# ForeverFancy/GVFDiffusion

Measured on AMD Instinct MI355X. Metric: 4D frames/sec (800x800x24f, 256k Gaussians) + DiT denoise steps/sec, higher is better.
Workload: dtype f32; 1 GPU; BASELINE configs[1]: single-GPU HIP rasteriser, one 4D sample per step = 24 frames x 800x800, 262144 Gaussians + per-frame deltas (fused activations), SH degree 2, mip 2D filter, white bg; gaussians=262144, resolution=800, sh_degree=2, parallelism=sample-sharded x1, samples_in_flight=2

## Files before the change

### gvfdiffusion_amd/csrc/rast.hip

```cpp
#include <atomic>
#include <cstdlib>
#include <vector>
#include "rast_common.h"
#include "gvf_sort.h"

namespace {

#ifndef GVF_PRE_FB
#define GVF_PRE_FB 4
#endif
constexpr int PRE_FB = GVF_PRE_FB;
#ifndef GVF_PRE_WAVE_FB
#define GVF_PRE_WAVE_FB 6
#endif
constexpr int PRE_WAVES = PRE_THREADS / GVF_WAVE;
constexpr int PRE_WAVE_FB = GVF_PRE_WAVE_FB;

struct PreParams {
    int P, M, deg, H, W, mode;
    int gx, gy;
    float kernel_size, scale_modifier;
    int fused;
    GvfGaussianActivation act;
    int n_delta;
    int upstream_binning;
    int F;
    int delta_lds;
};

__global__ __launch_bounds__(256) void activate_kernel(GvfGaussianActivation a, int P, int M,
                                                       const float* __restrict__ xyz_raw,
                                                       const float* __restrict__ features_dc,
                                                       const float* __restrict__ scaling_raw,
                                                       const float* __restrict__ rotation_raw,
                                                       const float* __restrict__ opacity_raw,
                                                       const float* __restrict__ delta, float* __restrict__ means3D,
                                                       float* __restrict__ scales, float* __restrict__ rotations,
                                                       float* __restrict__ shs, float* __restrict__ opacities) {
    int i = blockIdx.x * blockDim.x + threadIdx.x;
    if (i >= P) return;
    const float* d = delta ? delta + 14 * (size_t)i : nullptr;
    ActGaussian g = activate_one(i, a, xyz_raw, scaling_raw, rotation_raw, opacity_raw, d);
    for (int k = 0; k < 3; ++k) { means3D[3 * (size_t)i + k] = g.p[k]; scales[3 * (size_t)i + k] = g.s[k]; }
    for (int k = 0; k < 4; ++k) rotations[4 * (size_t)i + k] = g.q[k];
    opacities[i] = g.op;
    for (int m = 0; m < M; ++m)
        for (int c = 0; c < 3; ++c) {
            float v = features_dc[((size_t)i * M + m) * 3 + c];
            shs[((size_t)i * M + m) * 3 + c] = d ? v + g.drgb[c] : v;
        }
}

constexpr int ACT_MAX_SLICES = 16;
struct ActSlices { int n; int di[ACT_MAX_SLICES]; };
__global__ __launch_bounds__(256) void activate_cov_kernel(GvfGaussianActivation a, float scale_modifier, int P, ActSlices sl,
                                                           const float* __restrict__ xyz_raw, const float* __restrict__ scaling_raw,
                                                           const float* __restrict__ rotation_raw, const float* __restrict__ opacity_raw,
                                                           const float* __restrict__ delta, float4* __restrict__ rec3d,
                                                           const uint32_t* __restrict__ slot_of ,
                                                           const float* __restrict__ sh, int sh_floats, float* __restrict__ sh_by_slot) {
    const int i = blockIdx.x * blockDim.x + threadIdx.x;
    if (i >= P) return;
    const size_t dst = slot_of != nullptr ? (size_t)slot_of[i] : (size_t)i;
    if (sh_by_slot != nullptr && blockIdx.y == 0)
        for (int k = 0; k < sh_floats; ++k) sh_by_slot[dst * sh_floats + k] = sh[(size_t)i * sh_floats + k];
    const int di = sl.di[blockIdx.y];
    const float* d = (delta != nullptr && di >= 0) ? delta + ((size_t)di * P + i) * 14 : nullptr;
    const ActGaussian g = activate_one(i, a, xyz_raw, scaling_raw, rotation_raw, opacity_raw, d);
    float c6[6];
    cov3d_from_scale_rot(g.s, scale_modifier, g.q, c6);
    float4* r = rec3d + 4 * ((size_t)blockIdx.y * P + dst);
    r[0] = make_float4(g.p[0], g.p[1], g.p[2], g.op);
    r[1] = make_float4(c6[0], c6[1], c6[2], c6[3]);
    r[2] = make_float4(c6[4], c6[5], g.drgb[0], g.drgb[1]);
    r[3] = make_float4(g.drgb[2], 0.f, 0.f, 0.f);
}

__device__ __forceinline__ float ln_upper(float z) {
    const uint32_t b = __float_as_uint(z);
    const int e = (int)(b >> 23) - 127;
    const float m = __uint_as_float((b & 0x7fffffu) | 0x3f800000u);
    float L = (m - 1.0f) * 1.4426951f;
    L = fminf(L, 0.32192809f + (m - 1.25f) * 1.1541561f);
    L = fminf(L, 0.5849625f + (m - 1.5f) * 0.96179669f);
    L = fminf(L, 0.80735492f + (m - 1.75f) * 0.8243972f);
    L = fminf(L, 1.0f + (m - 2.0f) * 0.72134752f);
    return ((float)e + (L + 1e-5f)) * 0.69314724f;
}

__device__ __forceinline__ float2 cull_extent(float ca, float cb, float cc, float op) {
    if (op < 1.0f / 255.0f) return make_float2(-1.0f, -1.0f);
    const float det = ca * cc - cb * cb;
    const float inf = __builtin_inff();
    if (!(det > 0.0f) || !(ca > 0.0f) || !(cc > 0.0f)) return make_float2(inf, inf);
    const float tau = 2.0f * ln_upper(255.0f * op) * 1.001f + 1e-3f;
    const float inv = 1.0f / det;
    return make_float2(sqrtf(tau * cc * inv) * 1.001f + 0.01f, sqrtf(tau * ca * inv) * 1.001f + 0.01f);
}

__device__ __forceinline__ void tight_range(float c, float h, int lo, int hi, int n, int& t0, int& t1) {
    if (h < 0.0f) { t0 = lo; t1 = lo; return; }
    const float a = fminf(fmaxf(ceilf((c - h - (float)(TILE - 1)) / (float)TILE), 0.0f), (float)n);
    const float b = fminf(fmaxf(floorf((c + h) / (float)TILE) + 1.0f, 0.0f), (float)n);
    t0 = max((int)a, lo);
    t1 = min((int)b, hi);
    if (t1 < t0) t1 = t0;
}

__device__ __forceinline__ TileRect tight_rect(TileRect r, float px, float py, float hx, float hy, int gx, int gy) {
    TileRect t;
    tight_range(px, hx, r.x0, r.x1, gx, t.x0, t.x1);
    tight_range(py, hy, r.y0, r.y1, gy, t.y0, t.y1);
    return t;
}

template <bool SHARED, bool WAVE_FRAMES = false>
__global__ __launch_bounds__(PRE_THREADS) void preprocess_kernel(
    PreParams pp, const GvfRastFrame* __restrict__ frames, const float* __restrict__ a0,
    const float* __restrict__ a1, const float* __restrict__ a2, const float* __restrict__ a3,
    const float* __restrict__ sh, const float* __restrict__ colors_precomp,
    const float* __restrict__ cov3D_precomp, const float* __restrict__ delta, float4* __restrict__ splats,
    uint32_t* __restrict__ tiles_touched,
    int32_t* __restrict__ radii, uint32_t* __restrict__ block_sums, uint4* __restrict__ binrec,
    const uint32_t* __restrict__ bin_slot ) {
    static_assert(!(SHARED && WAVE_FRAMES), "the shared-activation launch keeps the 256-Gaussian mapping");
    extern __shared__ __attribute__((aligned(16))) float sh_lds[];
    constexpr int PRE_GPB = WAVE_FRAMES ? GVF_WAVE : PRE_THREADS;
    const int t = threadIdx.x;
    const int P = pp.P, M = pp.M;
    const int nbx = (P + PRE_THREADS - 1) / PRE_THREADS;
    const int bx = blockIdx.x, by = blockIdx.y;
    const int row = WAVE_FRAMES ? (t & (GVF_WAVE - 1)) : t;
    const int i = bx * PRE_GPB + row;

    const int sh_stride = M * 3;
    if (sh != nullptr) {
        const size_t span0 = (size_t)bx * PRE_GPB * sh_stride;
        const int nvalid = min(PRE_GPB, P - bx * PRE_GPB);
        const int total = nvalid * sh_stride;
        const float4* src4 = reinterpret_cast<const float4*>(sh + span0);
        float4* dst4 = reinterpret_cast<float4*>(sh_lds);
        const int n4 = total >> 2;
        for (int k = t; k < n4; k += PRE_THREADS) dst4[k] = src4[k];
        for (int k = (n4 << 2) + t; k < total; k += PRE_THREADS) sh_lds[k] = sh[span0 + k];
    }
    __syncthreads();

  const uint32_t my_slot = (bin_slot != nullptr && i < P) ? bin_slot[i] : (uint32_t)i;
  ActRaw raw = {};
  if (WAVE_FRAMES && pp.fused && i < P) raw = activate_raw(i, pp.act, a0, a1, a2, a3);
  const int f_first = WAVE_FRAMES ? by * (PRE_WAVES * PRE_WAVE_FB) + __builtin_amdgcn_readfirstlane(t >> 6) : by * PRE_FB;
  constexpr int F_STEP = WAVE_FRAMES ? PRE_WAVES : 1, F_COUNT = WAVE_FRAMES ? PRE_WAVE_FB : PRE_FB;
#pragma unroll 1
  for (int ff = 0; ff < F_COUNT; ++ff) {
    const int f = f_first + ff * F_STEP;
    if (f >= pp.F) break;
    const GvfRastFrame* fr = frames + f;
    uint32_t touched = 0;
    int radius_out = 0;
    float4 gA = make_float4(0.f, 0.f, 0.f, 0.f), gB = gA, gC = gA;
    TileRect rect = {0, 0, 0, 0};

    if (i < P) {
        float p[3], s[3], q[4], op, dadd[3] = {0.f, 0.f, 0.f};
        float c6s[6];
        if (SHARED) {
            const float4* r3 = reinterpret_cast<const float4*>(a0) + 4 * ((size_t)fr->reserved[0] * P + i);
            const float4 r0 = r3[0], r1 = r3[1], r2 = r3[2], r3v = r3[3];
            p[0] = r0.x; p[1] = r0.y; p[2] = r0.z; op = r0.w;
            c6s[0] = r1.x; c6s[1] = r1.y; c6s[2] = r1.z; c6s[3] = r1.w; c6s[4] = r2.x; c6s[5] = r2.y;
            dadd[0] = r2.z; dadd[1] = r2.w; dadd[2] = r3v.x;
        } else if (pp.fused) {
            const int di = fr->delta_index;
            const float* d = (delta != nullptr && di >= 0) ? delta + ((size_t)di * P + i) * 14 : nullptr;
            ActGaussian g;
            if (WAVE_FRAMES) {
                float dl[14];
#pragma unroll
                for (int k = 0; k < 14; ++k) dl[k] = d ? d[k] : 0.0f;
                g = activate_finish(raw, pp.act, dl, d != nullptr);
            } else {
                g = activate_one(i, pp.act, a0, a1, a2, a3, d);
            }
#pragma unroll
            for (int k = 0; k < 3; ++k) { p[k] = g.p[k]; s[k] = g.s[k]; dadd[k] = g.drgb[k]; }
#pragma unroll
            for (int k = 0; k < 4; ++k) q[k] = g.q[k];
            op = g.op;
        } else {
#pragma unroll
            for (int k = 0; k < 3; ++k) p[k] = a0[3 * (size_t)i + k];
            if (cov3D_precomp == nullptr) {
#pragma unroll
                for (int k = 0; k < 3; ++k) s[k] = a1[3 * (size_t)i + k];
#pragma unroll
                for (int k = 0; k < 4; ++k) q[k] = a2[4 * (size_t)i + k];
            }
            op = a3[i];
        }

        float pv[3];
        xform43(fr->viewmatrix, p, pv);
        bool vis = pv[2] > 0.2f;
        if (vis) {
            float ph[4];
            xform44(fr->projmatrix, p, ph);
            float pw = 1.0f / (ph[3] + 0.0000001f);
            float projx = ph[0] * pw, projy = ph[1] * pw;

            float c6[6];
            if (SHARED) {
#pragma unroll
                for (int k = 0; k < 6; ++k) c6[k] = c6s[k];
            } else if (!pp.fused && cov3D_precomp != nullptr) {
#pragma unroll
                for (int k = 0; k < 6; ++k) c6[k] = cov3D_precomp[6 * (size_t)i + k];
            } else {
                cov3d_from_scale_rot(s, pp.scale_modifier, q, c6);
            }

            const float tanfovx = fr->tanfovx, tanfovy = fr->tanfovy;
            float focal_x = (float)pp.W / (2.0f * tanfovx);
            float focal_y = (float)pp.H / (2.0f * tanfovy);
            float limx = 1.3f * tanfovx, limy = 1.3f * tanfovy;
            float txtz = pv[0] / pv[2], tytz = pv[1] / pv[2];
            float tx = fminf(limx, fmaxf(-limx, txtz)) * pv[2];
            float ty = fminf(limy, fmaxf(-limy, tytz)) * pv[2];
            float tz = pv[2];
            float J00 = focal_x / tz, J02 = -(focal_x * tx) / (tz * tz);
            float J11 = focal_y / tz, J12 = -(focal_y * ty) / (tz * tz);
            float A0[3], A1[3];
#pragma unroll
            for (int c = 0; c < 3; ++c) {
                float w0 = fr->viewmatrix[c * 4 + 0], w1 = fr->viewmatrix[c * 4 + 1], w2 = fr->viewmatrix[c * 4 + 2];
                A0[c] = J00 * w0 + J02 * w2;
                A1[c] = J11 * w1 + J12 * w2;
            }
            float S[3][3] = {{c6[0], c6[1], c6[2]}, {c6[1], c6[3], c6[4]}, {c6[2], c6[4], c6[5]}};
            float B0[3], B1[3];
#pragma unroll
            for (int c = 0; c < 3; ++c) {
                B0[c] = A0[0] * S[0][c] + A0[1] * S[1][c] + A0[2] * S[2][c];
                B1[c] = A1[0] * S[0][c] + A1[1] * S[1][c] + A1[2] * S[2][c];
            }
            float cxx = B0[0] * A0[0] + B0[1] * A0[1] + B0[2] * A0[2];
            float cxy = B0[0] * A1[0] + B0[1] * A1[1] + B0[2] * A1[2];
            float cyy = B1[0] * A1[0] + B1[1] * A1[1] + B1[2] * A1[2];

            float coef = 1.0f;
            if (pp.mode == GVF_RAST_MODE_MIP) {
                float det0 = fmaxf(1e-6f, cxx * cyy - cxy * cxy);
                float det1 = fmaxf(1e-6f, (cxx + pp.kernel_size) * (cyy + pp.kernel_size) - cxy * cxy);
                coef = sqrtf(det0 / (det1 + 1e-6f) + 1e-6f);
                if (det0 <= 1e-6f || det1 <= 1e-6f) coef = 0.0f;
                cxx += pp.kernel_size;
                cyy += pp.kernel_size;
            } else {
                cxx += 0.3f;
                cyy += 0.3f;
            }
            float det = cxx * cyy - cxy * cxy;
            if (det != 0.0f) {
                float det_inv = 1.f / det;
                float ca = cyy * det_inv, cb = -cxy * det_inv, cc = cxx * det_inv;
                float mid = 0.5f * (cxx + cyy);
                float lam1 = mid + sqrtf(fmaxf(0.1f, mid * mid - det));
                float lam2 = mid - sqrtf(fmaxf(0.1f, mid * mid - det));
                float my_radius = ceilf(3.f * sqrtf(fmaxf(lam1, lam2)));
                float px = ((projx + 1.0f) * (float)pp.W - 1.0f) * 0.5f;
                float py = ((projy + 1.0f) * (float)pp.H - 1.0f) * 0.5f;
                TileRect r = get_rect(px, py, my_radius, pp.gx, pp.gy);
                uint32_t cnt = (uint32_t)((r.x1 - r.x0) * (r.y1 - r.y0));
                if (cnt != 0) {
                    float rgb[3];
                    if (colors_precomp != nullptr) {
                        rgb[0] = colors_precomp[3 * (size_t)i + 0];
                        rgb[1] = colors_precomp[3 * (size_t)i + 1];
                        rgb[2] = colors_precomp[3 * (size_t)i + 2];
                    } else {
                        sh_to_rgb(pp.deg, sh_lds + row * sh_stride, dadd, p, fr->campos, rgb);
                    }
                    radius_out = (int)my_radius;
                    const float2 ext = cull_extent(ca, cb, cc, op * coef);
                    if (!pp.upstream_binning) {
                        r = tight_rect(r, px, py, ext.x, ext.y, pp.gx, pp.gy);
                        cnt = (uint32_t)((r.x1 - r.x0) * (r.y1 - r.y0));
                    }
                    touched = cnt;
                    rect = r;
                    gA = make_float4(px, py, ca * CONIC_K1, cb * CONIC_K2);
                    gB = make_float4(cc * CONIC_K1, op * coef, rgb[0], rgb[1]);
                    gC = make_float4(rgb[2], pv[2], ext.x, ext.y);
                }
            }
        }
        const size_t o = (size_t)f * P + i;
        if (!WAVE_FRAMES && tiles_touched != nullptr) tiles_touched[o] = touched;
        if (radii != nullptr) {
            const uint32_t* gid_of = SHARED ? reinterpret_cast<const uint32_t*>(a1) : nullptr;
            radii[gid_of != nullptr ? (size_t)f * P + gid_of[i] : o] = radius_out;
        }
        if (binrec != nullptr) {
            binrec[(size_t)f * P + my_slot] = make_uint4((uint32_t)rect.x0 | ((uint32_t)rect.y0 << 16),
                                                         (uint32_t)rect.x1 | ((uint32_t)rect.y1 << 16), __float_as_uint(gC.y), 0u);
        }
    }

    const int lj = t & 3;
    float4* qbase = splats + 4 * ((size_t)f * P + (size_t)(i & ~3));
#define GVF_QB(v_, k_) __builtin_bit_cast(float, __builtin_amdgcn_mov_dpp(__builtin_bit_cast(int, (v_)), (k_) * 0x55, 0xF, 0xF, true))
#define GVF_QSTORE(k_)                                                                                          \
    {                                                                                                       \
        const int tk = __builtin_amdgcn_mov_dpp((int)touched, (k_) * 0x55, 0xF, 0xF, true);                 \
        float4 o4;                                                                                          \
        { const float a = GVF_QB(gA.x, k_), b = GVF_QB(gB.x, k_), c = GVF_QB(gC.x, k_); o4.x = lj == 0 ? a : (lj == 1 ? b : (lj == 2 ? c : 0.f)); } \
        { const float a = GVF_QB(gA.y, k_), b = GVF_QB(gB.y, k_), c = GVF_QB(gC.y, k_); o4.y = lj == 0 ? a : (lj == 1 ? b : (lj == 2 ? c : 0.f)); } \
        { const float a = GVF_QB(gA.z, k_), b = GVF_QB(gB.z, k_), c = GVF_QB(gC.z, k_); o4.z = lj == 0 ? a : (lj == 1 ? b : (lj == 2 ? c : 0.f)); } \
        { const float a = GVF_QB(gA.w, k_), b = GVF_QB(gB.w, k_), c = GVF_QB(gC.w, k_); o4.w = lj == 0 ? a : (lj == 1 ? b : (lj == 2 ? c : 0.f)); } \
        if (tk != 0) qbase[4 * (k_) + lj] = o4;                                                             \
    }
    GVF_QSTORE(0) GVF_QSTORE(1) GVF_QSTORE(2) GVF_QSTORE(3)
#undef GVF_QSTORE
#undef GVF_QB

    if (!WAVE_FRAMES && block_sums != nullptr) {
        const unsigned lane = t & 63, w = t >> 6;
        uint32_t incl = gvf_wave_incl_scan(touched, lane);
        __shared__ uint32_t wsum[PRE_THREADS / GVF_WAVE];
        __syncthreads();
        if (lane == 63) wsum[w] = incl;
        __syncthreads();
        if (t == 0) block_sums[(size_t)f * nbx + bx] = wsum[0] + wsum[1] + wsum[2] + wsum[3];
    }
  }
}

__global__ __launch_bounds__(1024) void scan_sums_kernel(uint32_t* __restrict__ block_sums, int nb, int F,
                                                         uint32_t* __restrict__ frame_base ,
                                                         uint32_t* __restrict__ num_rendered ,
                                                         uint32_t* __restrict__ total_out, uint32_t max_rendered) {
    __shared__ uint32_t wsum[16];
    __shared__ uint32_t carry_s;
    const int t = threadIdx.x;
    const unsigned lane = t & 63, w = t >> 6;
    const int n = nb * F;
    if (t == 0) carry_s = 0;
    __syncthreads();
    for (int base = 0; base < n; base += 1024) {
        int j = base + t;
        uint32_t v = j < n ? block_sums[j] : 0u;
        uint32_t incl = gvf_wave_incl_scan(v, lane);
        if (lane == 63) wsum[w] = incl;
        __syncthreads();
        uint32_t wbase = 0, tot = 0;
        for (unsigned k = 0; k < 16; ++k) { if (k < w) wbase += wsum[k]; tot += wsum[k]; }
        uint32_t carry = carry_s;
        uint32_t excl = carry + wbase + incl - v;
        if (j < n) {
            block_sums[j] = excl;
            if (j % nb == 0) frame_base[j / nb] = excl;
        }
        __syncthreads();
        if (t == 0) carry_s = carry + tot;
        __syncthreads();
    }
    if (t == 0) { frame_base[F] = carry_s; *total_out = carry_s > max_rendered ? 0u : carry_s; }
    __syncthreads();
    for (int f = t; f < F; f += 1024) num_rendered[f] = frame_base[f + 1] - frame_base[f];
}

__global__ __launch_bounds__(PRE_THREADS) void duplicate_kernel(
    int P, int gx, int gy, const float4* __restrict__ splats,
    const uint32_t* __restrict__ tiles_touched, const int32_t* __restrict__ radii_ws,
    const uint32_t* __restrict__ block_base, uint64_t* __restrict__ keys, uint32_t* __restrict__ vals,
    uint32_t max_rendered, int upstream_binning) {
    __shared__ uint32_t wsum[PRE_THREADS / GVF_WAVE];
    const int t = threadIdx.x, f = blockIdx.y;
    const int i = blockIdx.x * PRE_THREADS + t;
    const unsigned lane = t & 63, w = t >> 6;
    const size_t o = (size_t)f * P + i;
    uint32_t touched = i < P ? tiles_touched[o] : 0u;
    uint32_t incl = gvf_wave_incl_scan(touched, lane);
    if (lane == 63) wsum[w] = incl;
    __syncthreads();
    uint32_t wbase = 0;
    for (unsigned k = 0; k < w; ++k) wbase += wsum[k];
    uint32_t off = block_base[(size_t)f * gridDim.x + blockIdx.x] + wbase + incl - touched;
    if (touched == 0) return;
    if ((uint64_t)off + touched > (uint64_t)max_rendered) return;
    const float4 a = splats[4 * o];
    const float4 c = splats[4 * o + 2];
    const float depth = c.y;
    TileRect r = get_rect(a.x, a.y, (float)radii_ws[o], gx, gy);
    if (!upstream_binning) r = tight_rect(r, a.x, a.y, c.z, c.w, gx, gy);
    const uint64_t tile0 = (uint64_t)f * (uint32_t)(gx * gy);
    const uint32_t dbits = __float_as_uint(depth);
    for (int y = r.y0; y < r.y1; ++y)
        for (int x = r.x0; x < r.x1; ++x) {
            uint64_t key = ((tile0 + (uint32_t)(y * gx + x)) << 32) | dbits;
            keys[off] = key;
            vals[off] = (uint32_t)i;
            ++off;
        }
}

__device__ __forceinline__ uint32_t float_ordered(float f) {
    const uint32_t u = __float_as_uint(f);
    return (u & 0x80000000u) ? ~u : (u | 0x80000000u);
}
__device__ __forceinline__ float float_unordered(uint32_t o) {
    return __uint_as_float((o & 0x80000000u) ? (o & 0x7fffffffu) : ~o);
}

constexpr int SCAN_CHUNK = 4096;
__global__ __launch_bounds__(1024) void seg_sums_kernel(const uint32_t* __restrict__ cnt, int n, uint32_t* __restrict__ partial) {
    __shared__ uint32_t wsum[16];
    const int t = threadIdx.x, j0 = blockIdx.x * SCAN_CHUNK + 4 * t;
    uint32_t s = 0;
#pragma unroll
    for (int k = 0; k < 4; ++k) s += j0 + k < n ? cnt[j0 + k] : 0u;
#pragma unroll
    for (int d = 32; d >= 1; d >>= 1) s += __shfl_xor(s, d, 64);
    if ((t & 63) == 0) wsum[t >> 6] = s;
    __syncthreads();
    if (t == 0) { uint32_t tot = 0; for (int k = 0; k < 16; ++k) tot += wsum[k]; partial[blockIdx.x] = tot; }
}

__global__ __launch_bounds__(1024) void seg_scan_kernel(const uint32_t* __restrict__ cnt, int n, int ntiles, int F,
                                                        const uint32_t* __restrict__ partial, int nblocks,
                                                        uint2* __restrict__ ranges, uint32_t* __restrict__ cursor,
                                                        uint32_t* __restrict__ frame_base ,
                                                        uint32_t* __restrict__ num_rendered ,
                                                        uint32_t* __restrict__ total_out, uint32_t max_rendered,
                                                        uint32_t* __restrict__ cls ) {
    __shared__ uint32_t wsum[16], wtot[16];
    __shared__ uint32_t s_base, s_total;
    const int t = threadIdx.x;
    const unsigned lane = t & 63, w = t >> 6;
    uint32_t before = 0, all = 0;
    for (int k = t; k < nblocks; k += 1024) { const uint32_t p = partial[k]; all += p; if (k < (int)blockIdx.x) before += p; }
#pragma unroll
    for (int d = 32; d >= 1; d >>= 1) { before += __shfl_xor(before, d, 64); all += __shfl_xor(all, d, 64); }
    if (lane == 0) { wsum[w] = before; wtot[w] = all; }
    __syncthreads();
    if (t == 0) {
        uint32_t b = 0, a = 0;
        for (int k = 0; k < 16; ++k) { b += wsum[k]; a += wtot[k]; }
        s_base = b; s_total = a;
    }
    __syncthreads();
    const uint32_t total = s_total;
    const bool overflow = total > max_rendered;
    const int j0 = blockIdx.x * SCAN_CHUNK + 4 * t;
    uint32_t c[4], s = 0;
#pragma unroll
    for (int k = 0; k < 4; ++k) { c[k] = j0 + k < n ? cnt[j0 + k] : 0u; s += c[k]; }
    const uint32_t incl = gvf_wave_incl_scan(s, lane);
    __syncthreads();
    if (lane == 63) wsum[w] = incl;
    __syncthreads();
    uint32_t run = s_base + incl - s;
    for (unsigned k = 0; k < w; ++k) run += wsum[k];
#pragma unroll
    for (int k = 0; k < 4; ++k) {
        const int j = j0 + k;
        if (j < n) {
            ranges[j] = overflow ? make_uint2(0u, 0u) : make_uint2(run, run + c[k]);
            cursor[j] = run;
            if (!overflow && c[k] > (uint32_t)SORT_SMALL_N) {
                if (c[k] > (uint32_t)SORT_LARGE_N) cls[2 + n + atomicAdd(&cls[1], 1u)] = (uint32_t)j;
                else cls[2 + atomicAdd(&cls[0], 1u)] = (uint32_t)j | (c[k] > (uint32_t)SORT_MEDIUM_N ? 0x80000000u : 0u);
            }
            if (j % ntiles == 0) frame_base[j / ntiles] = run;
        }
        run += c[k];
    }
// ... 243 lines not shown
        }
        if (k == n - 1) ranges[cur].y = n;
    }
}

struct FrameChunk { GvfRastFrame f[16]; };
struct CallTables {
    uint32_t* ranges; uint32_t n_ranges;
    uint32_t* tile_count; uint32_t n_tile_count;
    uint32_t* mhist; uint32_t n_mhist;
    uint32_t* cls;
    uint32_t* mm;
    uint32_t layout;
};
__global__ void upload_frames_kernel(FrameChunk c, int count, GvfRastFrame* __restrict__ dst, CallTables tab) {
    if (blockIdx.x == 0) {
        const int words = (int)(sizeof(GvfRastFrame) / 4) * count;
        const uint32_t* src = reinterpret_cast<const uint32_t*>(&c);
        for (int k = threadIdx.x; k < words; k += blockDim.x) reinterpret_cast<uint32_t*>(dst)[k] = src[k];
        if (tab.cls != nullptr && threadIdx.x < 2) tab.cls[threadIdx.x] = 0u;
        if (tab.mm != nullptr && threadIdx.x < 6) tab.mm[threadIdx.x] = threadIdx.x < 3 ? 0xffffffffu : 0u;
        if (tab.mm != nullptr && threadIdx.x == LAYOUT_WORD) tab.mm[LAYOUT_WORD] = tab.layout;
        return;
    }
    const uint32_t t = (blockIdx.x - 1) * blockDim.x + threadIdx.x, nt = (gridDim.x - 1) * blockDim.x;
    for (uint32_t k = t; k < tab.n_ranges; k += nt) tab.ranges[k] = 0u;
    for (uint32_t k = t; k < tab.n_tile_count; k += nt) tab.tile_count[k] = 0u;
    for (uint32_t k = t; k < tab.n_mhist; k += nt) tab.mhist[k] = 0u;
}

constexpr int PROF_MAX_CALLS = 256;
constexpr int PROF_EVENTS = GVF_RAST_NSTAGES + 1;
struct Profiler {
    bool on = false;
    std::atomic<int> calls{0};
    hipEvent_t ev[PROF_MAX_CALLS][PROF_EVENTS];
};
Profiler g_prof;
inline void prof_mark(hipStream_t s, int slot, int k) {
    if (slot >= 0) (void)hipEventRecord(g_prof.ev[slot][k], s);
}

int key_end_bit(int F, int ntiles) {
    uint64_t m = (uint64_t)F * (uint64_t)ntiles;
    int bits = 0;
    while (((uint64_t)1 << bits) < m) ++bits;
    return 32 + bits;
}

std::atomic<long long> g_shared_calls{0};

int run_pipeline(const GvfRastSettings& st, const GvfRastFrame* frames_host, int F, int P, int M, bool fused,
                 const GvfGaussianActivation* act, const float* a0, const float* a1, const float* a2,
                 const float* a3, const float* sh, const float* colors_precomp, const float* cov3D_precomp,
                 const float* delta, int n_delta, const float* subpixel_offset, void* workspace,
                 size_t workspace_bytes, int64_t max_rendered, float* out_color, float* out_alpha,
                 float* out_depth, int32_t* out_radii, uint32_t* out_num_rendered, hipStream_t stream,
                 unsigned char* out_u8 = nullptr ) {
    const int H = st.image_height, W = st.image_width;
    if (H <= 0 || W <= 0 || P < 0 || F <= 0 || max_rendered < 0 || max_rendered > 0xFFFFFFFFll) return GVF_EINVAL;
    if (st.sh_degree < 0 || st.sh_degree > 3) return GVF_EINVAL;
    if (st.mode != GVF_RAST_MODE_MIP && st.mode != GVF_RAST_MODE_DILATE) return GVF_EINVAL;
    if ((out_color == nullptr) == (out_u8 == nullptr) || !out_num_rendered || !frames_host || !workspace) return GVF_EINVAL;
    if (P > 0 && colors_precomp == nullptr) {
        if (sh == nullptr || M < (st.sh_degree + 1) * (st.sh_degree + 1) || M > MAX_SH_COEFFS) return GVF_EINVAL;
    }
    (void)hipGetLastError();
    if ((((uintptr_t)sh) & 15) != 0 || (((uintptr_t)workspace) & 255) != 0) return GVF_EINVAL;
    Workspace w = carve(workspace, workspace_bytes, P, F, H, W, max_rendered);
    if (!w.ok) return GVF_ENOSPC;

    const int gx = (W + TILE - 1) / TILE, gy = (H + TILE - 1) / TILE, ntiles = gx * gy;
    const int nb = (P + PRE_THREADS - 1) / PRE_THREADS;
    int slot = g_prof.on ? g_prof.calls.fetch_add(1) : -1;
    if (slot >= PROF_MAX_CALLS) slot = -1;

    ActSlices slices; slices.n = 0;
    bool shared = false;
    std::vector<int> frame_slice((size_t)F, 0);
    const char* shared_env = getenv("GVF_RAST_SHARED_ACT");
    const bool shared_on = !(shared_env && shared_env[0] == '0');
    const char* wf_env = getenv("GVF_RAST_PRE_WAVE_FRAMES");
    const bool wave_frames_on = !(wf_env && wf_env[0] == '0');
    if (shared_on && fused && cov3D_precomp == nullptr && st.bin_algo != GVF_RAST_BIN_RADIX && P > 0 && F >= 2) {
        shared = true;
        for (int f = 0; f < F && shared; ++f) {
            const int di = (delta != nullptr && frames_host[f].delta_index >= 0) ? frames_host[f].delta_index : -1;
            int k = 0;
            while (k < slices.n && slices.di[k] != di) ++k;
            if (k == slices.n) {
                if (slices.n == ACT_MAX_SLICES) { shared = false; break; }
                slices.di[slices.n++] = di;
            }
            frame_slice[(size_t)f] = k;
        }
        if (shared && (F < 2 * slices.n || (size_t)slices.n * (size_t)P * 64u > (size_t)(max_rendered > 0 ? max_rendered : 0) * 8u)) shared = false;
    }
    const bool index_count = st.bin_algo != GVF_RAST_BIN_RADIX && !shared && ntiles <= BINX_TAB;
    const bool morton = st.bin_algo != GVF_RAST_BIN_RADIX && F >= 4 && P >= 4096;
    const char* slot_env = getenv("GVF_RAST_SLOT_ORDER");
    const size_t sh_floats = (size_t)(colors_precomp ? 0 : M) * 3;
    const bool slot_mode = shared && !(slot_env && slot_env[0] == '0') && morton && nb > 0 && colors_precomp == nullptr && sh != nullptr &&
                           (size_t)slices.n * (size_t)P * 64u + (size_t)P * sh_floats * 4u <= (size_t)max_rendered * 8u;
    const uint32_t layout = slot_mode ? LAYOUT_SLOT_ORDER : 0u;
    for (int f0 = 0; f0 < F; f0 += 16) {
        FrameChunk ch;
        const int cnt = F - f0 < 16 ? F - f0 : 16;
        for (int k = 0; k < cnt; ++k) {
            ch.f[k] = frames_host[f0 + k];
            ch.f[k].reserved[0] = shared ? frame_slice[(size_t)(f0 + k)] : 0;
        }
        CallTables tab = {};
        if (f0 == 0) {
            const size_t nseg_all = (size_t)F * ntiles;
            tab.ranges = reinterpret_cast<uint32_t*>(w.ranges); tab.n_ranges = (uint32_t)(2 * nseg_all);
            tab.tile_count = w.tile_count; tab.n_tile_count = (uint32_t)nseg_all;
            tab.mhist = w.mhist; tab.n_mhist = morton ? (uint32_t)MORTON_BINS : 0u;
            tab.cls = w.cls; tab.mm = w.mm; tab.layout = layout;
        }
        const size_t clear_words = (size_t)tab.n_ranges + tab.n_tile_count + tab.n_mhist;
        const int zb = f0 == 0 ? (int)((clear_words + 4095) / 4096 < 256 ? (clear_words + 4095) / 4096 : 256) : 0;
        hipLaunchKernelGGL(upload_frames_kernel, dim3(1 + zb), dim3(256), 0, stream, ch, cnt, w.frames + f0, tab);
    }
    GVF_CHECK_LAUNCH();

    const uint32_t* blend_rec_of = nullptr;
    if (P == 0 || nb == 0) {
        if (hipMemsetAsync(out_num_rendered, 0, sizeof(uint32_t) * F, stream) != hipSuccess) return GVF_ELAUNCH;
    } else {
        const bool bucket = st.bin_algo != GVF_RAST_BIN_RADIX;
        prof_mark(stream, slot, 0);
        const uint32_t* order = nullptr;
        if (morton) {
            int bb = (P + 255) / 256; if (bb > 128) bb = 128;
            const int pb = (P + 255) / 256;
            hipLaunchKernelGGL(bbox_kernel, dim3(bb), dim3(256), 0, stream, P, a0, w.mm);
            hipLaunchKernelGGL(morton_count_kernel, dim3(pb), dim3(256), 0, stream, P, a0, w.mm, w.order_alt, w.mhist);
            hipLaunchKernelGGL(morton_scan_kernel, dim3(1), dim3(1024), 0, stream, w.mhist);
            hipLaunchKernelGGL(morton_scatter_kernel, dim3(pb), dim3(256), 0, stream, P, w.order_alt, w.mhist, w.order);
            order = w.order;
            GVF_CHECK_LAUNCH();
        }
        const bool rec_gather = bucket && !shared && order != nullptr;
        const unsigned nseg = (unsigned)((size_t)F * ntiles);
        prof_mark(stream, slot, 1);
        PreParams pp;
        pp.P = P; pp.M = colors_precomp ? 0 : M; pp.deg = st.sh_degree; pp.H = H; pp.W = W; pp.mode = st.mode;
        pp.gx = gx; pp.gy = gy; pp.kernel_size = st.kernel_size; pp.scale_modifier = st.scale_modifier;
        pp.fused = fused ? 1 : 0; pp.n_delta = n_delta; pp.F = F;
        pp.upstream_binning = (st.upstream_binning != 0 || subpixel_offset != nullptr) ? 1 : 0;
        if (fused) pp.act = *act; else pp.act = GvfGaussianActivation{};
        const size_t sh_lds_bytes = gvf_align_up((size_t)PRE_THREADS * pp.M * 3 * sizeof(float), 16) + 16;
        pp.delta_lds = 0;
        const dim3 pre_grid(nb, (F + PRE_FB - 1) / PRE_FB);
        if (shared) {
            g_shared_calls.fetch_add(1, std::memory_order_relaxed);
            float4* rec3d = reinterpret_cast<float4*>(w.keys_alt);
            float* sh_by_slot = slot_mode ? reinterpret_cast<float*>(rec3d + 4 * (size_t)slices.n * (size_t)P) : nullptr;
            hipLaunchKernelGGL(activate_cov_kernel, dim3((P + 255) / 256, slices.n), dim3(256), 0, stream, *act, st.scale_modifier, P, slices,
                               a0, a1, a2, a3, delta, rec3d, slot_mode ? w.order_alt : nullptr, sh, (int)sh_floats, sh_by_slot);
            if (slot_mode) {
                blend_rec_of = w.order_alt;
                hipLaunchKernelGGL(preprocess_kernel<true>, pre_grid, dim3(PRE_THREADS), sh_lds_bytes, stream, pp,
                                   w.frames, reinterpret_cast<const float*>(rec3d), reinterpret_cast<const float*>(order), nullptr, nullptr, sh_by_slot,
                                   nullptr, nullptr, nullptr, w.splats, nullptr, out_radii == nullptr ? nullptr : w.radii, nullptr, w.binrec, nullptr);
            } else
            hipLaunchKernelGGL(preprocess_kernel<true>, pre_grid, dim3(PRE_THREADS), sh_lds_bytes, stream, pp,
                               w.frames, reinterpret_cast<const float*>(rec3d), nullptr, nullptr, nullptr, colors_precomp ? nullptr : sh, colors_precomp,
                               nullptr, nullptr, w.splats, nullptr, out_radii == nullptr ? nullptr : w.radii, nullptr, w.binrec,
                               order != nullptr ? w.order_alt : nullptr);
        } else if (bucket && wave_frames_on) {
            const size_t wf_lds_bytes = gvf_align_up((size_t)GVF_WAVE * pp.M * 3 * sizeof(float), 16) + 16;
            const dim3 wf_grid((P + GVF_WAVE - 1) / GVF_WAVE, (F + PRE_WAVES * PRE_WAVE_FB - 1) / (PRE_WAVES * PRE_WAVE_FB));
            hipLaunchKernelGGL((preprocess_kernel<false, true>), wf_grid, dim3(PRE_THREADS), wf_lds_bytes, stream, pp,
                               w.frames, a0, a1, a2, a3, colors_precomp ? nullptr : sh, colors_precomp, cov3D_precomp, delta,
                               w.splats, nullptr, out_radii == nullptr ? nullptr : w.radii, nullptr, w.binrec, nullptr);
        } else
        hipLaunchKernelGGL(preprocess_kernel<false>, pre_grid, dim3(PRE_THREADS), sh_lds_bytes, stream, pp,
                           w.frames, a0, a1, a2, a3, colors_precomp ? nullptr : sh, colors_precomp, cov3D_precomp, delta,
                           w.splats, bucket ? nullptr : w.tiles_touched, (bucket && out_radii == nullptr) ? nullptr : w.radii,
                           bucket ? nullptr : w.block_sums, bucket ? w.binrec : nullptr, nullptr);
        const int bnb = (P + BIN_SLOTS - 1) / BIN_SLOTS, xnb = (P + BINX_PER_WG - 1) / BINX_PER_WG;
        const dim3 bin_grid = rec_gather ? dim3((unsigned)((F + 7) / 8 * 8 * bnb)) : dim3(bnb, F);
        if (index_count)
            hipLaunchKernelGGL(bin_index_kernel, dim3(xnb, F), dim3(BINX_THREADS), 0, stream, P, gx, w.binrec,
                               w.tile_count, w.cursor, w.total, w.keys, ntiles, nullptr, nullptr);
        else if (bucket)
            hipLaunchKernelGGL(bin_kernel<false>, bin_grid, dim3(PRE_THREADS), 0, stream, P, gx, gy, w.binrec, order,
                               w.tile_count, w.cursor, w.total, w.keys, nullptr, nullptr, rec_gather ? 1 : 0, rec_gather ? 1 : 0, F);
        GVF_CHECK_LAUNCH();
        prof_mark(stream, slot, 2);
        if (bucket)
        {
            const int sblocks = (int)((nseg + SCAN_CHUNK - 1) / SCAN_CHUNK);
            hipLaunchKernelGGL(seg_sums_kernel, dim3(sblocks), dim3(1024), 0, stream, w.tile_count, (int)nseg, w.partial);
            hipLaunchKernelGGL(seg_scan_kernel, dim3(sblocks), dim3(1024), 0, stream, w.tile_count, (int)nseg, ntiles, F,
                               w.partial, sblocks, w.ranges, w.cursor, w.frame_base, out_num_rendered, w.total,
                               (uint32_t)max_rendered, w.cls);
            if (max_rendered <= 0)
                hipLaunchKernelGGL(frame_counts_kernel, dim3((F + 63) / 64), dim3(64), 0, stream, w.frame_base, F, out_num_rendered);
        }
        else
            hipLaunchKernelGGL(scan_sums_kernel, dim3(1), dim3(1024), 0, stream, w.block_sums, nb, F, w.frame_base,
                               out_num_rendered, w.total, (uint32_t)max_rendered);
        GVF_CHECK_LAUNCH();
        prof_mark(stream, slot, 3);
        if (max_rendered > 0) {
            if (bucket)
                hipLaunchKernelGGL(bin_kernel<true>, bin_grid, dim3(PRE_THREADS), 0, stream, P, gx, gy, w.binrec, order,
                                   w.tile_count, w.cursor, w.total, w.keys, w.frame_base, out_num_rendered,
                                   rec_gather ? 1 : 0, rec_gather ? 1 : 0, F);
            else
                hipLaunchKernelGGL(duplicate_kernel, dim3(nb, F), dim3(PRE_THREADS), 0, stream, P, gx, gy, w.splats,
                                   w.tiles_touched, w.radii, w.block_sums, w.keys, w.vals, (uint32_t)max_rendered,
                                   pp.upstream_binning);
            GVF_CHECK_LAUNCH();
        }
        if (out_radii != nullptr) {
            if (hipMemcpyAsync(out_radii, w.radii, sizeof(int32_t) * (size_t)F * P, hipMemcpyDeviceToDevice, stream) != hipSuccess)
                return GVF_ELAUNCH;
        }
        prof_mark(stream, slot, 4);
        if (max_rendered > 0) {
            uint64_t* keys_sorted = w.keys;
            uint32_t* vals_by_tile = nullptr;
            if (!bucket) {
                vals_by_tile = w.vals;
                int in_alt = 0;
                int rc = gvf_sort_pairs_device_n(w.keys, w.keys_alt, w.vals, w.vals_alt, w.total, max_rendered, 32,
                                                 key_end_bit(F, ntiles), w.sort_tmp, w.sort_tmp_bytes, stream, &in_alt);
                if (rc != GVF_OK) return rc;
                if (in_alt) { keys_sorted = w.keys_alt; vals_by_tile = w.vals_alt; }
                int rblocks = (int)((max_rendered + 255) / 256);
                if (rblocks > 4096) rblocks = 4096;
                hipLaunchKernelGGL(ranges_kernel, dim3(rblocks), dim3(256), 0, stream, keys_sorted, w.total,
                                   (uint32_t)max_rendered, w.ranges, (uint32_t)nseg);
                GVF_CHECK_LAUNCH();
            }
            prof_mark(stream, slot, 5);
            const int rc = launch_tile_sort(stream, w.ranges, keys_sorted, vals_by_tile, w.ids, w.cls, nseg, bucket ? 2 : 1);
            if (rc != GVF_OK) return rc;
        } else {
            prof_mark(stream, slot, 5);
        }
    }
    const char* order_env = getenv("GVF_RAST_BLEND_ORDER");
    const bool order_tiles = !(order_env && order_env[0] == '0') && P > 0 && nb > 0 && max_rendered > 0 && (size_t)F * ntiles >= 2048;
    const int rc = launch_blend(stream, st, P, F, w.ranges, w.ids, w.splats, subpixel_offset, out_color, out_alpha, out_depth, out_u8,
                                blend_rec_of, order_tiles ? w.cursor : nullptr, slot >= 0 ? g_prof.ev[slot][6] : nullptr);
    if (rc != GVF_OK) return rc;
    prof_mark(stream, slot, 7);
    return GVF_OK;
}

}

Workspace gvf_rast::carve(void* ws, size_t bytes, int P, int F, int H, int W, int64_t max_rendered) {
    Workspace w;
    GvfCarver c(ws, bytes);
    const int nb = (P + PRE_THREADS - 1) / PRE_THREADS;
    const int ntiles = ((W + TILE - 1) / TILE) * ((H + TILE - 1) / TILE);
    const size_t FP = (size_t)F * (size_t)(P > 0 ? P : 1);
    const size_t D = (size_t)(max_rendered > 0 ? max_rendered : 1);
    w.frames = c.take<GvfRastFrame>(F);
    w.splats = c.take<float4>(4 * FP);
    w.tiles_touched = c.take<uint32_t>(FP);
    w.radii = c.take<int32_t>(FP);
    w.block_sums = c.take<uint32_t>((size_t)F * (nb > 0 ? nb : 1));
    w.frame_base = c.take<uint32_t>(F + 1);
    w.total = c.take<uint32_t>(1);
    w.keys = c.take<uint64_t>(D);
    w.keys_alt = c.take<uint64_t>(D);
    w.vals = c.take<uint32_t>(D);
    w.vals_alt = c.take<uint32_t>(D);
    w.ids = c.take<uint32_t>(D);
    w.ranges = c.take<uint2>((size_t)F * ntiles);
    w.cls = c.take<uint32_t>(2 + 2 * (size_t)F * ntiles);
    w.tile_count = c.take<uint32_t>((size_t)F * ntiles);
    w.cursor = c.take<uint32_t>((size_t)F * ntiles);
    w.partial = c.take<uint32_t>(((size_t)F * ntiles + SCAN_CHUNK - 1) / SCAN_CHUNK + 1);
    const size_t Pp = (size_t)(P > 0 ? P : 1);
    w.order = c.take<uint32_t>(Pp);
    w.order_alt = c.take<uint32_t>(Pp);
    w.mhist = c.take<uint32_t>(1 << 15);
    w.mm = c.take<uint32_t>(8);
    w.binrec = c.take<uint4>(FP);
    w.sort_tmp_bytes = gvf_sort_tmp_bytes((int64_t)D);
    w.sort_tmp = c.take<char>(w.sort_tmp_bytes);
    w.bytes = gvf_align_up(c.off, 256);
    w.ok = c.ok;
    return w;
}

extern "C" int gvf_rast_workspace_bytes(int P, int F, int H, int W, int64_t max_rendered, size_t* bytes) {
    if (!bytes || P < 0 || F <= 0 || H <= 0 || W <= 0 || max_rendered < 0) return GVF_EINVAL;
    Workspace w = carve(nullptr, (size_t)-1, P, F, H, W, max_rendered);
    *bytes = w.bytes + 256;
    (void)tile_sort_set_lds_limit();
    return GVF_OK;
}

extern "C" int gvf_rast_forward(const GvfRastSettings* st, const GvfRastFrame* frame_host, int P, int M,
                                const float* means3D, const float* shs, const float* colors_precomp,
                                const float* opacities, const float* scales, const float* rotations,
                                const float* cov3D_precomp, const float* subpixel_offset, void* workspace,
                                size_t workspace_bytes, int64_t max_rendered, float* out_color, float* out_alpha,
                                float* out_depth, int32_t* out_radii, uint32_t* out_num_rendered, void* stream) {
    if (!st || !frame_host) return GVF_EINVAL;
    if (P > 0) {
        if (!means3D || !opacities) return GVF_EINVAL;
        if ((shs == nullptr) == (colors_precomp == nullptr)) return GVF_EINVAL;
        const bool have_sr = scales != nullptr && rotations != nullptr;
        if (have_sr == (cov3D_precomp != nullptr)) return GVF_EINVAL;
    }
    return run_pipeline(*st, frame_host, 1, P, M, false, nullptr, means3D, scales, rotations, opacities, shs,
                        colors_precomp, cov3D_precomp, nullptr, 0, subpixel_offset, workspace, workspace_bytes,
                        max_rendered, out_color, out_alpha, out_depth, out_radii, out_num_rendered,
                        (hipStream_t)stream);
}

extern "C" int gvf_rast_forward_batched(const GvfRastSettings* st, const GvfRastFrame* frames_host, int F,
                                        const GvfGaussianActivation* act, int P, int M, const float* xyz_raw,
                                        const float* features_dc, const float* scaling_raw,
                                        const float* rotation_raw, const float* opacity_raw, const float* delta,
                                        int n_delta, void* workspace, size_t workspace_bytes,
// ... 100 lines not shown
```

Before: 21370 frames/s.

## Prefetch per-frame deltas into LDS via async global_load_lds double buffering

In the wave-frames preprocess path, the 14-float per-Gaussian delta rows for upcoming frames are staged into a per-wave LDS slab using global_load_lds DMA instructions, issued one or two frames ahead. The current frame's deltas are then read from registers filled out of LDS instead of from strided global loads. The goal is to hide global memory latency for the delta reads and to replace uncoalesced 56-byte row loads with coalesced bulk transfers. The cost is extra LDS per block, waitcnt synchronisation, and compiler barriers that may affect scheduling. There is an env switch to disable it.

```diff
diff --git a/gvfdiffusion_amd/csrc/rast.hip b/gvfdiffusion_amd/csrc/rast.hip
--- a/gvfdiffusion_amd/csrc/rast.hip
+++ b/gvfdiffusion_amd/csrc/rast.hip
@@ -27,6 +27,12 @@
     int F;
     int delta_lds;
 };
+
+#ifndef GVF_PRE_DELTA_DMA_AHEAD
+#define GVF_PRE_DELTA_DMA_AHEAD 1
+#endif
+constexpr int PRE_DELTA_ROW_BYTES = 14 * (int)sizeof(float);
+constexpr int PRE_DELTA_SLAB_BYTES = GVF_WAVE * PRE_DELTA_ROW_BYTES;
 
 __global__ __launch_bounds__(256) void activate_kernel(GvfGaussianActivation a, int P, int M,
                                                        const float* __restrict__ xyz_raw,
@@ -151,11 +157,60 @@
   if (WAVE_FRAMES && pp.fused && i < P) raw = activate_raw(i, pp.act, a0, a1, a2, a3);
   const int f_first = WAVE_FRAMES ? by * (PRE_WAVES * PRE_WAVE_FB) + __builtin_amdgcn_readfirstlane(t >> 6) : by * PRE_FB;
   constexpr int F_STEP = WAVE_FRAMES ? PRE_WAVES : 1, F_COUNT = WAVE_FRAMES ? PRE_WAVE_FB : PRE_FB;
+
+  constexpr bool DMA_AHEAD = GVF_PRE_DELTA_DMA_AHEAD != 0;
+  unsigned char* const slab = reinterpret_cast<unsigned char*>(sh_lds) + pp.delta_lds + (WAVE_FRAMES ? f_first - by * (PRE_WAVES * PRE_WAVE_FB) : 0) * PRE_DELTA_SLAB_BYTES;
+  const bool dma_group = WAVE_FRAMES && pp.delta_lds != 0 && pp.fused && delta != nullptr && P - bx * PRE_GPB >= PRE_GPB;
+  auto dma_span = [&](int f) -> const float* {
+      if (!dma_group || f >= pp.F) return nullptr;
+      const int di = frames[f].delta_index;
+      if (di < 0) return nullptr;
+      const float* span = delta + ((size_t)di * P + (size_t)bx * PRE_GPB) * 14;
+      return (reinterpret_cast<uintptr_t>(span) & 15) == 0 ? span : nullptr;
+  };
+  static_assert(PRE_DELTA_SLAB_BYTES == 3 * 1024 + 2 * 256, "three 1-KiB and two 256-byte instructions");
+  auto dma_issue = [&](const float* span) {
+      __attribute__((address_space(3))) void* dst = (__attribute__((address_space(3))) void*)slab;
+      __builtin_amdgcn_global_load_lds(span + 4 * row, dst, 16, 0, 0);
+      __builtin_amdgcn_global_load_lds(span + 4 * row, dst, 16, 1024, 0);
+      __builtin_amdgcn_global_load_lds(span + 4 * row, dst, 16, 2048, 0);
+      __builtin_amdgcn_global_load_lds(span + row, dst, 4, 3072, 0);
+      __builtin_amdgcn_global_load_lds(span + row, dst, 4, 3328, 0);
+  };
+  auto dma_read = [&](float (&dl)[14]) {
+      asm volatile("s_waitcnt vmcnt(0)" ::: "memory");
+      const float2* r = reinterpret_cast<const float2*>(slab + row * PRE_DELTA_ROW_BYTES);
+#pragma unroll
+      for (int k = 0; k < 7; ++k) { const float2 v = r[k]; dl[2 * k] = v.x; dl[2 * k + 1] = v.y; }
+      asm volatile("s_waitcnt lgkmcnt(0)" ::: "memory");
+  };
+  float dnx[14] = {};
+  bool cur_staged = false;
+  bool nxt_pending = false;
+  if (WAVE_FRAMES && DMA_AHEAD) {
+      const float* s0 = dma_span(f_first);
+      cur_staged = s0 != nullptr;
+      if (cur_staged) { dma_issue(s0); dma_read(dnx); }
+      const float* s1 = F_COUNT > 1 ? dma_span(f_first + F_STEP) : nullptr;
+      nxt_pending = s1 != nullptr;
+      if (nxt_pending) dma_issue(s1);
+  }
 #pragma unroll 1
   for (int ff = 0; ff < F_COUNT; ++ff) {
     const int f = f_first + ff * F_STEP;
     if (f >= pp.F) break;
     const GvfRastFrame* fr = frames + f;
+    const float* span2 = nullptr;
+    if (WAVE_FRAMES && DMA_AHEAD && ff + 2 < F_COUNT) span2 = dma_span(f + 2 * F_STEP);
+    if (WAVE_FRAMES && !DMA_AHEAD) {
+        const float* s0 = dma_span(f);
+        cur_staged = s0 != nullptr;
+        if (cur_staged) { dma_issue(s0); dma_read(dnx); }
+        else {
+#pragma unroll
+            for (int k = 0; k < 14; ++k) asm volatile("" : "=v"(dnx[k]));
+        }
+    }
     uint32_t touched = 0;
     int radius_out = 0;
     float4 gA = make_float4(0.f, 0.f, 0.f, 0.f), gB = gA, gC = gA;
@@ -176,8 +231,15 @@
             ActGaussian g;
             if (WAVE_FRAMES) {
                 float dl[14];
-#pragma unroll
-                for (int k = 0; k < 14; ++k) dl[k] = d ? d[k] : 0.0f;
+                if (cur_staged) {
+#pragma unroll
+                    for (int k = 0; k < 14; ++k) dl[k] = dnx[k];
+                } else {
+#pragma unroll
+                    for (int k = 0; k < 14; ++k) dl[k] = d ? d[k] : 0.0f;
+#pragma unroll
+                    for (int k = 0; k < 14; ++k) asm volatile("" : "+v"(dl[k]));
+                }
                 g = activate_finish(raw, pp.act, dl, d != nullptr);
             } else {
                 g = activate_one(i, pp.act, a0, a1, a2, a3, d);
@@ -197,6 +259,17 @@
                 for (int k = 0; k < 4; ++k) q[k] = a2[4 * (size_t)i + k];
             }
             op = a3[i];
+            if (WAVE_FRAMES) {
+#pragma unroll
+                for (int k = 0; k < 3; ++k) asm volatile("" : "+v"(p[k]));
+                if (cov3D_precomp == nullptr) {
+#pragma unroll
+                    for (int k = 0; k < 3; ++k) asm volatile("" : "+v"(s[k]));
+#pragma unroll
+                    for (int k = 0; k < 4; ++k) asm volatile("" : "+v"(q[k]));
+                }
+                asm volatile("" : "+v"(op));
+            }
         }
 
         float pv[3];
@@ -277,6 +350,10 @@
                         rgb[0] = colors_precomp[3 * (size_t)i + 0];
                         rgb[1] = colors_precomp[3 * (size_t)i + 1];
                         rgb[2] = colors_precomp[3 * (size_t)i + 2];
+                        if (WAVE_FRAMES) {
+#pragma unroll
+                            for (int k = 0; k < 3; ++k) asm volatile("" : "+v"(rgb[k]));
+                        }
                     } else {
                         sh_to_rgb(pp.deg, sh_lds + row * sh_stride, dadd, p, fr->campos, rgb);
                     }
@@ -294,6 +371,15 @@
                 }
             }
         }
+        if (WAVE_FRAMES && DMA_AHEAD) {
+            if (nxt_pending) {
+                dma_read(dnx);
+            } else {
+#pragma unroll
+                for (int k = 0; k < 14; ++k) asm volatile("" : "=v"(dnx[k]));
+            }
+            if (span2 != nullptr) dma_issue(span2);
+        }
         const size_t o = (size_t)f * P + i;
         if (!WAVE_FRAMES && tiles_touched != nullptr) tiles_touched[o] = touched;
         if (radii != nullptr) {
@@ -322,6 +408,7 @@
     GVF_QSTORE(0) GVF_QSTORE(1) GVF_QSTORE(2) GVF_QSTORE(3)
 #undef GVF_QSTORE
 #undef GVF_QB
+    if (WAVE_FRAMES && DMA_AHEAD) { cur_staged = nxt_pending; nxt_pending = span2 != nullptr; }
 
     if (!WAVE_FRAMES && block_sums != nullptr) {
         const unsigned lane = t & 63, w = t >> 6;
@@ -871,6 +958,8 @@
         if (fused) pp.act = *act; else pp.act = GvfGaussianActivation{};
         const size_t sh_lds_bytes = gvf_align_up((size_t)PRE_THREADS * pp.M * 3 * sizeof(float), 16) + 16;
         pp.delta_lds = 0;
+        const char* dma_env = getenv("GVF_RAST_PRE_DELTA_DMA");
+        const bool delta_dma_on = !(dma_env && dma_env[0] == '0');
         const dim3 pre_grid(nb, (F + PRE_FB - 1) / PRE_FB);
         if (shared) {
             g_shared_calls.fetch_add(1, std::memory_order_relaxed);
@@ -889,7 +978,11 @@
                                nullptr, nullptr, w.splats, nullptr, out_radii == nullptr ? nullptr : w.radii, nullptr, w.binrec,
                                order != nullptr ? w.order_alt : nullptr);
         } else if (bucket && wave_frames_on) {
-            const size_t wf_lds_bytes = gvf_align_up((size_t)GVF_WAVE * pp.M * 3 * sizeof(float), 16) + 16;
+            size_t wf_lds_bytes = gvf_align_up((size_t)GVF_WAVE * pp.M * 3 * sizeof(float), 16) + 16;
+            if (delta_dma_on && fused && delta != nullptr) {
+                pp.delta_lds = (int)wf_lds_bytes;
+                wf_lds_bytes += (size_t)PRE_WAVES * PRE_DELTA_SLAB_BYTES;
+            }
             const dim3 wf_grid((P + GVF_WAVE - 1) / GVF_WAVE, (F + PRE_WAVES * PRE_WAVE_FB - 1) / (PRE_WAVES * PRE_WAVE_FB));
             hipLaunchKernelGGL((preprocess_kernel<false, true>), wf_grid, dim3(PRE_THREADS), wf_lds_bytes, stream, pp,
                                w.frames, a0, a1, a2, a3, colors_precomp ? nullptr : sh, colors_precomp, cov3D_precomp, delta,
```

Measured after the change: 21700 frames/s (median of 6 runs). 1.5% higher.
